# bystrogenomics/bystro-vcf

Hardware: NVIDIA B200
Metric: variants/s (higher is better)
Workload: dtype u8

## Files before the change

### bystro_vcf_b200/csrc/bvcf_api.cu

```cuda
#include "../../include/bvcf.h"

#include <algorithm>
#include <chrono>
#include <cstdio>
#include <cstdlib>
#include <cstring>
#include <string>
#include <vector>

#include "bvcf_common.cuh"
#include "bvcf_prefix.cuh"
#include "bvcf_rows.cuh"
#include "bvcf_tile.cuh"
#include "bvcf_names.cuh"
#include "bvcf_scan.cuh"
#include "bvcf_inflate.cuh"
#include "bvcf_deflate.cuh"

using namespace bvcf;

namespace {

struct DevBuf {
  void *p = nullptr;
// ... 155 lines not shown
  if ((rc = dev_reserve(ctx, sc.tile_base, max_tiles * sizeof(TileBase)))) return rc;
  if ((rc = dev_reserve(ctx, sc.tile_partial, (size_t)TSCAN_BLOCKS * TQ * 8))) return rc;
  sc.scratch_cap = std::max<uint64_t>(sc.scratch_cap, std::min<uint64_t>(total_bytes / 8 + (8ull << 20), sc.max_records * 224ull + (1ull << 20)));
  if ((rc = dev_reserve(ctx, sc.tile_scratch, sc.scratch_cap + 64))) return rc;
  sc.slow_cap = std::max<uint32_t>(sc.slow_cap, 1u << 16);
  if ((rc = dev_reserve(ctx, sc.slow, (size_t)sc.slow_cap * sizeof(SlowRec)))) return rc;
  if (ctx->dcfg.n_samples > 0) {
    sc.row_cap = std::max<uint64_t>(sc.row_cap, sc.max_records / 2 + 1024);
    if ((rc = dev_reserve(ctx, sc.stats1, sc.max_records * sizeof(LineStats)))) return rc;
    if ((rc = dev_reserve(ctx, sc.row_desc, sc.row_cap * sizeof(RowDesc)))) return rc;
    if ((rc = dev_reserve(ctx, sc.big_recs, sc.max_records * 4))) return rc;
  }
  return 0;
}
void scratch_free(Scratch &sc) {
  for (DevBuf *b : {&sc.recs, &sc.range_nrec, &sc.range_nlines, &sc.rec_base, &sc.line_base, &sc.events, &sc.dense,
                    &sc.partial, &sc.stats1, &sc.row_desc, &sc.big_recs, &sc.tile_agg, &sc.tile_base, &sc.tile_partial,
                    &sc.tile_scratch, &sc.slow})
    dev_free(*b);
}

constexpr int N_STAGE_EV = 8;
struct StageEvents {
  cudaEvent_t e[N_STAGE_EV];
};

int enqueue_pipeline(bvcf_ctx *ctx, Scratch &sc, cudaStream_t st, const uint8_t *d_in, uint64_t begin, uint64_t len, uint64_t buf_len,
                     uint8_t *d_out, uint64_t out_cap, RunCounters *d_ctr, int8_t *d_dosage, uint64_t dosage_cap_rows,
                     uint8_t *d_loci, uint64_t loci_cap, unsigned long long *d_loci_off, uint32_t *d_diags,
                     uint32_t diag_cap, std::vector<StageEvents> *timing) {
  const DevCfg &dc = ctx->dcfg;
  const uint64_t a0 = begin & ~511ull;
  const uint64_t total_ranges = (len - a0 + sc.range_bytes - 1) / sc.range_bytes;
  int smem = SCAN_WARPS * RING;
  if (const char *e = getenv("BVCF_SCAN_SMEM_KB")) smem = std::max(smem, atoi(e) * 1024);
  cudaFuncSetAttribute(bvcf_scan_genotype_kernel<true>, cudaFuncAttributeMaxDynamicSharedMemorySize, smem);
  cudaFuncSetAttribute(bvcf_scan_genotype_kernel<false>, cudaFuncAttributeMaxDynamicSharedMemorySize, smem);
  int n_sm = 148;
  cudaDeviceGetAttribute(&n_sm, cudaDevAttrMultiProcessorCount, ctx->device);
  for (uint64_t r0 = 0; r0 < total_ranges; r0 += sc.n_ranges) {
    const uint32_t nr = (uint32_t)std::min<uint64_t>(sc.n_ranges, total_ranges - r0);
    StageEvents *se = nullptr;
    if (timing) {
      timing->emplace_back();
      se = &timing->back();
      for (int i = 0; i < N_STAGE_EV; i++) {
        if (ctx->ev_pool.empty()) {
          cudaEvent_t e;
          CK(cudaEventCreate(&e));
          se->e[i] = e;
        } else {
          se->e[i] = ctx->ev_pool.back();
          ctx->ev_pool.pop_back();
        }
      }
      CK(cudaEventRecord(se->e[0], st));
    }
    ScanParams sp{};
    sp.in = d_in; sp.begin = begin; sp.end = len; sp.buf_len = buf_len; sp.a0 = a0;
    sp.range_bytes = sc.range_bytes; sp.r0 = (uint32_t)r0; sp.n_ranges = nr;
    sp.slots_per_range = sc.slots; sp.evcap_words = sc.evcap_words;
    sp.recs = (LineRec *)sc.recs.p; sp.range_nrec = (uint32_t *)sc.range_nrec.p;
    sp.range_nlines = (uint32_t *)sc.range_nlines.p; sp.events = (uint32_t *)sc.events.p;
    sp.ctr = d_ctr; sp.H = dc.H; sp.eol_width = dc.eol_width;
    const unsigned grid = (nr + SCAN_WARPS - 1) / SCAN_WARPS;
    if (dc.n_samples > 0)
      bvcf_scan_genotype_kernel<true><<<grid, SCAN_WARPS * 32, smem, st>>>(sp);
    else
      bvcf_scan_genotype_kernel<false><<<grid, SCAN_WARPS * 32, smem, st>>>(sp);
    ctx->launches++;
    if (se) CK(cudaEventRecord(se->e[1], st));
    PrefixParams pp{};
    pp.a = sp.range_nrec; pp.b = sp.range_nlines;
    pp.out_a = (uint64_t *)sc.rec_base.p; pp.out_b = (uint64_t *)sc.line_base.p;
    pp.partial = (unsigned long long *)sc.partial.p;
    pp.n_ptr = nullptr; pp.n_imm = nr; pp.ctr = d_ctr;
    bvcf_prefix_reduce_kernel<<<PFX_BLOCKS, PFX_THREADS, 0, st>>>(pp);
    bvcf_prefix_spine_kernel<<<1, 1024, 0, st>>>(pp);
    bvcf_prefix_scan_kernel<<<PFX_BLOCKS, PFX_THREADS, 0, st>>>(pp);
    CompactParams cp{};
    cp.recs = sp.recs; cp.range_nrec = sp.range_nrec; cp.rec_base = pp.out_a; cp.line_base = pp.out_b;
    cp.dense = (LineRec *)sc.dense.p; cp.n_ranges = nr; cp.slots_per_range = sc.slots; cp.evcap_words = sc.evcap_words;
    bvcf_compact_lines_kernel<<<(nr + 7) / 8, 256, 0, st>>>(cp);
    ctx->launches += 4;
    if (se) CK(cudaEventRecord(se->e[2], st));
    const unsigned wgrid = (unsigned)n_sm * 64;
    if (dc.n_samples > 0) {
      StatsParams tp{};
      tp.in = d_in; tp.cfg = dc; tp.lines = cp.dense; tp.events = sp.events; tp.stats = (LineStats *)sc.stats1.p; tp.ctr = d_ctr;
      tp.big_recs = (uint32_t *)sc.big_recs.p;
      bvcf_line_stats_kernel<<<wgrid, 256, 0, st>>>(tp);
      bvcf_line_stats_big_kernel<<<(unsigned)n_sm * 4, 256, 0, st>>>(tp);
      ctx->launches += 2;
    }
    if (se) CK(cudaEventRecord(se->e[3], st));
    static const bool no_vec = getenv("BVCF_NO_NAMES_VEC") != nullptr;
    const bool vec = (dc.name8 || dc.name16) && dc.want_tsv && !no_vec && dc.n_samples > 0;
    TileParams tp{};
    tp.in = d_in; tp.cfg = dc; tp.lines = cp.dense; tp.events = sp.events; tp.stats = (const LineStats *)sc.stats1.p;
    tp.out = d_out; tp.out_cap = out_cap; tp.ctr = d_ctr;
    tp.tile_agg = (TileAgg *)sc.tile_agg.p; tp.tile_base = (TileBase *)sc.tile_base.p;
    tp.tile_partial = (unsigned long long *)sc.tile_partial.p;
    tp.scratch = (uint8_t *)sc.tile_scratch.p; tp.scratch_cap = sc.scratch_cap;
    tp.slow = (SlowRec *)sc.slow.p; tp.slow_cap = sc.slow_cap;
    tp.row_desc = (RowDesc *)sc.row_desc.p; tp.row_desc_cap = dc.n_samples > 0 ? sc.row_cap : 0;
    tp.long_words = vec ? 8192u : 0u;
    {
      static const int mid_q = getenv("BVCF_MID_QUADS") ? atoi(getenv("BVCF_MID_QUADS")) : 16;
      tp.mid_words = (dc.want_tsv && dc.n_samples > 0) ? 2u * (uint32_t)std::max(mid_q, 0) : 0u;
      if (!vec) tp.mid_words = 0;
    }
    tp.dosage = d_dosage; tp.dosage_cap_rows = dosage_cap_rows;
    tp.loci = d_loci; tp.loci_cap = loci_cap; tp.loci_off = d_loci_off;
    tp.diag.diags = d_diags; tp.diag.cap = diag_cap; tp.diag.ctr = d_ctr;
// ... 964 lines not shown
```

### bystro_vcf_b200/csrc/bvcf_common.cuh

```cuda
#pragma once
#include <cstdint>
#include <cuda_runtime.h>

namespace bvcf {

constexpr uint32_t FULL = 0xFFFFFFFFu;

struct __align__(16) LineRec {
  uint64_t start;
  uint32_t len;
  uint32_t an;
  uint32_t ev_start;
  uint32_t ev_count;
  uint32_t ord;
  uint16_t tab[9];
  uint16_t flags;
  uint32_t n_het1, n_hom1, n_miss, ac1;
};
static_assert(sizeof(LineRec) == 64, "LineRec layout");

constexpr uint32_t EV_SAMPLE_MASK = 0xFFFFFu;
constexpr uint32_t EV_COMPLEX = 1u << 30;
constexpr uint32_t EV_OFFSET_TAG = 1u << 31;
constexpr uint32_t EV_CODE_ABSENT = 30, EV_CODE_MISSING = 31;
constexpr uint32_t EV_NIB_MISSING = 0xEu, EV_NIB_ABSENT = 0xFu;
constexpr uint32_t EV_BASE_BIAS = 3;
constexpr uint32_t MAX_SAMPLES = (1u << 20) - 16;

__device__ __forceinline__ uint32_t ev_make(uint32_t sample, uint32_t c1, uint32_t c2) {
  return sample | (c1 << 20) | (c2 << 25);
}
__device__ __forceinline__ uint32_t ev_single_payload(uint32_t c1, uint32_t c2) {
  const uint32_t n1 = c1 == EV_CODE_MISSING ? EV_NIB_MISSING : c1;
  const uint32_t n2 = c2 == EV_CODE_MISSING ? EV_NIB_MISSING : (c2 == EV_CODE_ABSENT ? EV_NIB_ABSENT : c2);
  return n1 | (n2 << 16);
}
__device__ __forceinline__ uint32_t ev_slot_word(uint32_t h, uint32_t pl, int j) {
  const uint32_t samp = (h & EV_SAMPLE_MASK) + (uint32_t)j - EV_BASE_BIAS;
  if (h & EV_COMPLEX) return j == 0 ? (samp | EV_COMPLEX) : EV_OFFSET_TAG;
  const uint32_t n1 = (pl >> (4 * j)) & 0xFu, n2 = (pl >> (16 + 4 * j)) & 0xFu;
  if ((n1 | n2) == 0) return EV_OFFSET_TAG;
  if (n1 == EV_NIB_MISSING || n2 == EV_NIB_MISSING) return ev_make(samp, EV_CODE_MISSING, EV_CODE_MISSING);
  return ev_make(samp, n1, n2 == EV_NIB_ABSENT ? EV_CODE_ABSENT : n2);
}

struct RunCounters {
  unsigned long long out_cursor;
  unsigned long long row_cursor;
  unsigned long long loci_cursor;
  unsigned long long n_lines;
  unsigned long long n_records;
  unsigned long long chunk_out_base;
  unsigned long long chunk_row_base;
  unsigned long long chunk_loci_base;
  unsigned long long chunk_line_base;
  unsigned long long scratch_cursor;
  unsigned int ev_overflow;
  unsigned int slot_overflow;
  unsigned int out_overflow;
  unsigned int row_overflow;
  unsigned int n_diags;
  unsigned int chunk_records;
  unsigned int n_big_recs;
  unsigned int big_rec_cursor;
  unsigned int tile_ticket;
  unsigned int tile_ticket2;
  unsigned int n_slow;
  unsigned int scratch_overflow;
  unsigned int slow_overflow;
  unsigned int n_mid_rows;
  unsigned int n_big_rows;
  unsigned int big_row_cursor;
  unsigned int n_long_rows;
  unsigned int long_row_cursor;
};

struct DevCfg {
  int H;
  int n_samples;
  int eol_width;
  int keep_id, keep_info, keep_pos, want_tsv, want_dosage;
  int allow_all;
  int n_allow, n_excl;
  const uint8_t *filt_blob;
  const uint32_t *filt_off;
  int filt_bytes;
  uint8_t empty[64];
  int empty_len;
  uint8_t delim[64];
  int delim_len;
  uint8_t tail0[208];
  int tail0_len;
  const uint8_t *names;
  const uint32_t *name_off;
  int name_fixed_w;
  const unsigned long long *name8;
  const uint4 *name16;
  int item_bytes;
};

__device__ __forceinline__ uint32_t warp_incl_scan(uint32_t v, int lane) {
#pragma unroll
  for (int d = 1; d < 32; d <<= 1) {
    uint32_t t = __shfl_up_sync(FULL, v, d);
    if (lane >= d) v += t;
  }
  return v;
}
__device__ __forceinline__ uint32_t warp_sum(uint32_t v) {
#pragma unroll
  for (int d = 16; d > 0; d >>= 1) v += __shfl_xor_sync(FULL, v, d);
  return v;
}
__device__ __forceinline__ unsigned long long warp_sum64(unsigned long long v) {
#pragma unroll
  for (int d = 16; d > 0; d >>= 1) v += __shfl_xor_sync(FULL, v, d);
  return v;
}

__device__ __forceinline__ uint32_t eq_mask4(uint32_t w, uint32_t pat) {
  uint32_t t = w ^ pat;
  uint32_t y = (t & 0x7F7F7F7Fu) + 0x7F7F7F7Fu;
  y = ~(y | t | 0x7F7F7F7Fu);
  return ((y >> 7) * 0x00204081u >> 21) & 0xFu;
}
__device__ __forceinline__ uint32_t eq_mask16(const uint4 &v, uint32_t pat) {
  return eq_mask4(v.x, pat) | (eq_mask4(v.y, pat) << 4) | (eq_mask4(v.z, pat) << 8) | (eq_mask4(v.w, pat) << 12);
}

}
```

### bystro_vcf_b200/csrc/bvcf_prefix.cuh

```cuda
#pragma once
#include "bvcf_common.cuh"

namespace bvcf {

constexpr int PFX_BLOCKS = 592;
constexpr int PFX_THREADS = 256;

struct PrefixParams {
  const uint32_t *a, *b;
  uint64_t *out_a, *out_b;
  unsigned long long *partial;
  const unsigned int *n_ptr;
  uint32_t n_imm;
  RunCounters *ctr;
};

__device__ __forceinline__ uint32_t pfx_n(const PrefixParams &p) { return p.n_ptr ? *p.n_ptr : p.n_imm; }

__device__ __forceinline__ void pfx_span(uint32_t n, uint32_t &lo, uint32_t &hi) {
  const uint32_t span = (n + PFX_BLOCKS - 1) / PFX_BLOCKS;
  const unsigned long long l = (unsigned long long)blockIdx.x * span;
  lo = l > n ? n : (uint32_t)l;
  hi = l + span > n ? n : (uint32_t)(l + span);
}
// ... 65 lines not shown
  unsigned long long run_a = p.partial[2 * blockIdx.x], run_b = p.partial[2 * blockIdx.x + 1];
  const int w = threadIdx.x >> 5, l = threadIdx.x & 31;
  for (uint32_t base = lo; base < hi; base += PFX_THREADS) {
    const uint32_t i = base + threadIdx.x;
    const unsigned long long va = i < hi ? p.a[i] : 0, vb = (i < hi && p.b) ? p.b[i] : 0;
    unsigned long long ia = va, ib = vb;
#pragma unroll
    for (int d = 1; d < 32; d <<= 1) {
      const unsigned long long ta = __shfl_up_sync(FULL, ia, d), tb = __shfl_up_sync(FULL, ib, d);
      if (l >= d) { ia += ta; ib += tb; }
    }
    __syncthreads();
    if (l == 31) { wa[w] = ia; wb[w] = ib; }
    __syncthreads();
    unsigned long long oa = 0, ob = 0, ta = 0, tb = 0;
#pragma unroll
    for (int k = 0; k < PFX_THREADS / 32; k++) {
      if (k < w) { oa += wa[k]; ob += wb[k]; }
      ta += wa[k]; tb += wb[k];
    }
    if (i < hi) {
      p.out_a[i] = run_a + oa + ia - va;
      if (p.out_b) p.out_b[i] = run_b + ob + ib - vb;
    }
    run_a += ta; run_b += tb;
  }
}

struct CompactParams {
  const LineRec *recs;
  const uint32_t *range_nrec;
  const uint64_t *rec_base;
  const uint64_t *line_base;
  LineRec *dense;
  uint32_t n_ranges, slots_per_range, evcap_words;
};

__global__ void __launch_bounds__(256) bvcf_compact_lines_kernel(const CompactParams p) {
  const uint32_t r = blockIdx.x * 8 + (threadIdx.x >> 5);
  const int lane = threadIdx.x & 31;
  if (r >= p.n_ranges) return;
  uint32_t n = p.range_nrec[r];
  if (n > p.slots_per_range) n = p.slots_per_range;
  const LineRec *src = p.recs + (size_t)r * p.slots_per_range;
  LineRec *dst = p.dense + p.rec_base[r];
  const uint32_t lb = (uint32_t)p.line_base[r];
  for (uint32_t j = lane; j < n; j += 32) {
    LineRec x = src[j];
    x.ev_start += r * p.evcap_words;
    x.ord += lb;
    dst[j] = x;
  }
}

}
```

### bystro_vcf_b200/csrc/bvcf_rows.cuh

```cuda
#pragma once
#include "bvcf_common.cuh"
#include "bvcf_text.cuh"

namespace bvcf {

constexpr int NAMES_WARPS = 2;
constexpr int FILT_SMEM = 1024;

struct GtStats {
  uint32_t n_het, n_hom, n_miss, ac, an;
  uint32_t het_bytes, hom_bytes, miss_bytes;
};

constexpr int STAT_ALLELES = 3;
struct __align__(16) LineStats {
  uint32_t n_miss, an, miss_bytes, pad;
  uint32_t n_het[STAT_ALLELES], n_hom[STAT_ALLELES], ac[STAT_ALLELES], het_bytes[STAT_ALLELES], hom_bytes[STAT_ALLELES];
  uint32_t pad2;
};

struct __align__(16) RowDesc {
  uint32_t line;
  uint32_t allele;
  unsigned long long het_dst, hom_dst, miss_dst;
// ... 87 lines not shown
  const uint32_t q = v >> 2;
  off = 0;
  if (2 * q + 1 >= n_words) return EV_OFFSET_TAG;
  const uint2 e = *reinterpret_cast<const uint2 *>(ev + 2 * q);
  off = e.y;
  return ev_slot_word(e.x, e.y, (int)(v & 3u));
}

__device__ __forceinline__ int classify_word(uint32_t w, uint32_t off, const uint8_t *L,
                                             uint32_t content_len, uint32_t a, uint32_t &samp, uint32_t &gt_extra,
                                             uint32_t &alt) {
  gt_extra = 0; alt = 0; samp = 0;
  if (w & EV_OFFSET_TAG) return 0;
  samp = w & EV_SAMPLE_MASK;
  if (w & EV_COMPLEX) {
    uint32_t gt;
    const int cls = classify_gt_general(L + off, content_len > off ? content_len - off : 0, a, gt, alt);
    gt_extra = gt;
    return cls;
  }
  const uint32_t c1 = (w >> 20) & 31, c2 = (w >> 25) & 31;
  if (c1 == EV_CODE_MISSING) return 3;
  alt = (c1 == a) + (c2 == a);
  const uint32_t gt = c2 == EV_CODE_ABSENT ? 1 : 2;
  return alt == 0 ? 0 : (alt == gt ? 2 : 1);
}
__device__ __forceinline__ int classify_event(const uint32_t *ev, uint32_t v, uint32_t n_words, const uint8_t *L,
                                              uint32_t content_len, uint32_t a, uint32_t &samp, uint32_t &gt_extra,
                                              uint32_t &alt, bool &is_ev) {
  uint32_t off;
  const uint32_t w = slot_load(ev, v, n_words, off);
  is_ev = !(w & EV_OFFSET_TAG);
  return classify_word(w, off, L, content_len, a, samp, gt_extra, alt);
}

__device__ __forceinline__ uint32_t nib_eq(uint32_t x, uint32_t pat) {
  const uint32_t y = x ^ pat;
  return ~(((y & 0x77777777u) + 0x77777777u) | y) & 0x88888888u;
}

__device__ __forceinline__ void quad_masks(uint32_t h, uint32_t pl, uint32_t a, bool simple, const uint8_t *L,
                                           uint32_t content_len, bool valid, uint32_t &mh, uint32_t &mo, uint32_t &mm) {
  mh = mo = mm = 0;
  if (!valid) return;
  uint32_t one1, one2, dot, hap;
  if (simple) {
    const uint32_t b0 = pl << 3, b3 = pl;
    const uint32_t one = b0 & ~b3 & 0x88888888u, dt = b3 & ~b0 & 0x88888888u;
    one1 = one & 0x8888u; one2 = one >> 16;
    dot = dt | (dt >> 16);
    hap = (b3 & b0 & 0x88888888u) >> 16;
  } else {
    if (h & EV_COMPLEX) {
      uint32_t gt, alt;
      const int cls = classify_gt_general(L + pl, content_len > pl ? content_len - pl : 0, a, gt, alt);
      if (cls == 1) mh = 8u; else if (cls == 2) mo = 8u; else if (cls == 3) mm = 8u;
      return;
    }
    const uint32_t eq = a <= 9 ? nib_eq(pl, a * 0x11111111u) : 0u;
    const uint32_t dt = nib_eq(pl, 0xEEEEEEEEu);
    one1 = eq & 0x8888u; one2 = eq >> 16;
    dot = dt | (dt >> 16);
    hap = nib_eq(pl, 0xFFFFFFFFu) >> 16;
  }
  mm = dot & 0x8888u;
  mo = one1 & (one2 | hap) & ~mm;
  mh = (one1 ^ one2) & ~hap & ~mm & 0x8888u;
}

struct StatsParams {
  const uint8_t *in;
// ... 567 lines not shown
```

### bystro_vcf_b200/csrc/bvcf_scan.cuh

```cuda
#pragma once
#include "bvcf_common.cuh"

namespace bvcf {

constexpr int WIN = 512;
constexpr int STAGES = 8;
constexpr int RING = WIN * STAGES;
constexpr int PF_PAIRS = 3;
constexpr int SCAN_WARPS = 8;
constexpr int FS_NONE = 0x7FFFFFFF;

struct ScanParams {
  const uint8_t *in;
  uint64_t begin, end;
  uint64_t buf_len;
  uint64_t a0;
  uint32_t range_bytes;
  uint32_t r0, n_ranges;
  uint32_t slots_per_range, evcap_words;
  LineRec *recs;
  uint32_t *range_nrec;
  uint32_t *range_nlines;
  uint32_t *events;
  RunCounters *ctr;
  int H, eol_width;
};

struct LineAcc {
  uint32_t an_l, an_uni;
  uint32_t het_l, hom_l;
  uint32_t ac_l;
  uint32_t miss_l;
  uint32_t flag_l;
};

struct WarpState {
  uint64_t line_start;
  int fsr;
  uint32_t col;
  uint32_t ev_w, line_ev_start;
  uint32_t nrec, nlines;
  uint32_t refpat;
  int mode;
  LineAcc a;
};

__device__ __forceinline__ uint4 lds128(uint32_t a) {
  uint4 v;
  asm volatile("ld.shared.v4.u32 {%0,%1,%2,%3}, [%4];\n" : "=r"(v.x), "=r"(v.y), "=r"(v.z), "=r"(v.w) : "r"(a));
  return v;
}
__device__ __forceinline__ uint32_t lds32(uint32_t a) {
  uint32_t v;
  asm volatile("ld.shared.u32 %0, [%1];\n" : "=r"(v) : "r"(a));
  return v;
}

__device__ __forceinline__ uint32_t bits_range16(int lo, int hi) {
  lo = lo < 0 ? 0 : lo;
  hi = hi > 16 ? 16 : hi;
  return hi <= lo ? 0u : (((1u << hi) - 1u) & ~((1u << lo) - 1u));
}

__device__ __forceinline__ uint32_t tok_code(uint32_t c) {
  uint32_t d = c - '0';
  return c == '.' ? EV_CODE_MISSING : (d <= 9 ? d : 0u);
}

__device__ __forceinline__ void start_line(WarpState &st, uint64_t start, int rel) {
  st.line_start = start; st.fsr = rel; st.col = 0;
  st.a.an_l = st.a.an_uni = st.a.het_l = st.a.hom_l = st.a.ac_l = st.a.miss_l = st.a.flag_l = 0;
  st.line_ev_start = st.ev_w;
}

__device__ __forceinline__ void acc_sample(LineAcc &a, uint32_t c1, uint32_t c2) {
  const uint32_t hap = c2 == EV_CODE_ABSENT;
  const uint32_t alt = (c1 == 1) + (c2 == 1);
  a.ac_l += alt;
  a.hom_l += hap ? alt : (alt >> 1);
  a.het_l += hap ? 0u : (alt & 1u);
  a.flag_l |= (c1 > 1) | (!hap && c2 > 1);
}

__device__ __forceinline__ uint32_t pack_quad(const uint32_t t[4], bool dots) {
  if (dots) {
    const uint32_t K = 0x000F000Fu;
    return (t[0] & K) | ((t[1] & K) << 4) | ((t[2] & K) << 8) | ((t[3] & K) << 12);
  }
  return t[0] | (t[1] << 4) | (t[2] << 8) | (t[3] << 12);
}
__device__ __forceinline__ void acc_quad(LineAcc &a, uint32_t pl, bool dots) {
  const uint32_t y = pl ^ 0x11111111u;
  uint32_t one = ~(((y & 0x77777777u) + 0x77777777u) | y) & 0x88888888u;
  uint32_t big = pl & 0xEEEEEEEEu;
  if (dots) {
    const uint32_t d = pl ^ 0xEEEEEEEEu;
    const uint32_t dot = ~(((d & 0x77777777u) + 0x77777777u) | d) & 0x88888888u;
    const uint32_t mf = (dot | (dot >> 16)) & 0x8888u;
    const uint32_t nm = __popc(mf);
    a.miss_l += nm;
    a.an_l -= 2 * nm;
    const uint32_t gone = ((mf | (mf << 16)) >> 3) * 15u;
    one &= ~gone;
    big &= ~gone;
  }
  const uint32_t both = one & (one >> 16);
  const uint32_t n1 = __popc(one), n2 = __popc(both);
  a.ac_l += n1;
  a.hom_l += n2;
  a.het_l += n1 - 2 * n2;
  a.flag_l |= big;
}
__device__ __forceinline__ void classify_push_words4(const ScanParams &p, WarpState &st, uint32_t *my_events,
                                                     const uint32_t t[4], int samp0, bool dots, int lane) {
  const uint32_t pl = pack_quad(t, dots);
  const uint32_t bal = __ballot_sync(FULL, pl != 0);
  if (bal == 0) return;
  const uint32_t n = 2 * __popc(bal);
  if (st.ev_w + n <= p.evcap_words) {
    if (pl)
      *reinterpret_cast<uint2 *>(my_events + st.ev_w + 2 * __popc(bal & ((1u << lane) - 1u))) =
          make_uint2((uint32_t)(samp0 + (int)EV_BASE_BIAS), pl);
  } else if (lane == 0) {
    p.ctr->ev_overflow = 1;
  }
  if (pl) acc_quad(st.a, pl, dots);
  st.ev_w += n;
}

__device__ __forceinline__ void classify_push_pair(const ScanParams &p, WarpState &st, uint32_t *my_events,
                                                   const uint32_t ta[4], const uint32_t tb[4], int samp0, bool dots,
                                                   int lane) {
  const uint32_t pa = pack_quad(ta, dots), pb = pack_quad(tb, dots);
  const uint32_t ba = __ballot_sync(FULL, pa != 0), bb = __ballot_sync(FULL, pb != 0);
  if ((ba | bb) == 0) return;
  const uint32_t na = 2 * __popc(ba), n = na + 2 * __popc(bb);
  const uint32_t lt = (1u << lane) - 1u;
  if (st.ev_w + n <= p.evcap_words) {
    uint32_t *dst = my_events + st.ev_w;
    if (pa) *reinterpret_cast<uint2 *>(dst + 2 * __popc(ba & lt)) = make_uint2((uint32_t)(samp0 + (int)EV_BASE_BIAS), pa);
    if (pb)
      *reinterpret_cast<uint2 *>(dst + na + 2 * __popc(bb & lt)) = make_uint2((uint32_t)(samp0 + 128 + (int)EV_BASE_BIAS), pb);
  } else if (lane == 0) {
    p.ctr->ev_overflow = 1;
  }
  if (pa) acc_quad(st.a, pa, dots);
  if (pb) acc_quad(st.a, pb, dots);
  st.ev_w += n;
}

__device__ __forceinline__ uint32_t bad_digits4(const uint32_t t[4], uint32_t keep_mask3) {
  const uint32_t o = t[0] | t[1] | t[2] | (t[3] & keep_mask3);
  return (o & 0xFFF0FFF0u) | (((o & 0x000F000Fu) + 0x00060006u) & 0x00100010u);
}
__device__ __forceinline__ uint32_t bad_digits8(const uint32_t ta[4], const uint32_t tb[4]) {
  const uint32_t o = ta[0] | ta[1] | ta[2] | ta[3] | tb[0] | tb[1] | tb[2] | tb[3];
  return (o & 0xFFF0FFF0u) | (((o & 0x000F000Fu) + 0x00060006u) & 0x00100010u);
}
__device__ __forceinline__ uint32_t bad_digits_or_dots4(const uint32_t t[4], uint32_t keep_mask3) {
  const uint32_t o = t[0] | t[1] | t[2] | (t[3] & keep_mask3);
  uint32_t acc = 0;
#pragma unroll
  for (int j = 0; j < 4; j++) {
    const uint32_t x = t[j] + 0x00160016u, y = t[j] + 0x00020002u, z = t[j] + 0x00010001u;
    acc |= (x & ~y) | z;
  }
  return (o & 0xFFE0FFE0u) | (acc & 0x00200020u);
}

template <bool HAS_SAMPLES>
__device__ __forceinline__ void scan_window_general(const ScanParams &p, WarpState &st, uint32_t ring_base_s,
                                                    uint32_t stage_off, const uint4 &v, uint64_t pos, uint64_t rend,
                                                    int lane, LineRec *my_recs, uint32_t *my_events) {
  const bool eol2 = p.eol_width == 2;
  const uint32_t tm = eq_mask16(v, 0x09090909u);
  uint32_t nm = eq_mask16(v, 0x0A0A0A0Au);

  int seg_lo = 0;
  if (st.mode == 1 && st.fsr != FS_NONE && st.fsr > 0) {
    seg_lo = st.fsr;
    nm &= bits_range16(seg_lo - lane * 16, 16);
  }

  while (seg_lo < WIN) {
    const int lo_l = seg_lo - lane * 16;
    const uint32_t ball = __ballot_sync(FULL, nm != 0);
    int nl = WIN;
    if (ball) {
      const int l = __ffs(ball) - 1;
      const uint32_t m = __shfl_sync(FULL, nm, l);
      nl = l * 16 + __ffs(m) - 1;
      if (lane == l) nm &= nm - 1;
    }
    if (st.mode == 0) {
      if (nl == WIN) return;
      const uint64_t start = pos + nl + 1;
      if (start >= rend) { st.mode = 2; return; }
      st.mode = 1;
      start_line(st, start, nl + 1);
      seg_lo = nl + 1;
      continue;
    }
    int tab_hi = nl;
    if (eol2 && nl < WIN && nl > 0) tab_hi = nl - 1;
    const uint32_t tm_l = tm & bits_range16(lo_l, tab_hi - lane * 16);
    const uint32_t cnt = __popc(tm_l);
// ... 66 lines not shown
            bad_shape = true;
          }
        }
        uint32_t bad = bad_digits4(t, 0xFFFFFFFFu) | (bad_shape ? 1u : 0u);
        bool dots = false;
        if (!__all_sync(FULL, bad == 0)) {
          bad = bad_digits_or_dots4(t, 0xFFFFFFFFu) | (bad_shape ? 1u : 0u);
          dots = true;
        }
        if (__all_sync(FULL, bad == 0)) {
          vector_ok = true;
          const int samp0 = (int)samp_base + ((ws0 - s9) >> 2);
          st.a.an_l += 2 * __popc(zone);
          classify_push_words4(p, st, my_events, t, samp0, dots, lane);
          if (nl == WIN) {
            const int n_words = (WIN - s9 + 3) >> 2;
            const int ws_last = s9 + 4 * (n_words - 1);
            nfs = ws_last + 4 - WIN;
            col_extra = ws_last + 3 >= WIN ? 1u : 0u;
          }
        }
      }
      if (!vector_ok) {
        if (!have_excl) excl = warp_incl_scan(cnt, lane) - cnt;
        int last_end = -1;
        uint32_t last_sep = 0;
        const uint32_t prev_hi = __shfl_up_sync(FULL, tm_l >> 15, 1);
        uint32_t fm = ((tm_l << 1) | (lane > 0 ? (prev_hi & 1u) : 0u)) & 0xFFFFu;
        if (st.fsr == seg_lo) {
          const int sl = seg_lo - lane * 16;
          if (sl >= 0 && sl < 16) fm |= 1u << sl;
        }
        const uint32_t fm_all = fm;
        uint32_t evbuf[16];
        int nev = 0;
        while (fm) {
          const int sl = __ffs(fm) - 1;
          fm &= fm - 1;
          const uint32_t fidx = st.col + excl + __popc(tm_l & ((1u << sl) - 1u));
          last_end = -1;
          if (fidx < 9) continue;
          const uint32_t samp = fidx - 9;
          const int s = lane * 16 + sl;
          const uint32_t a = stage_off + (uint32_t)s;
          const uint32_t w0 = lds32(ring_base_s + ((a & ~3u) & (RING - 1)));
          const uint32_t w1 = lds32(ring_base_s + (((a & ~3u) + 4u) & (RING - 1)));
          const uint32_t sh = (a & 3u) * 8u;
          const uint32_t lo = __funnelshift_r(w0, w1, sh);
          const uint32_t b0 = lo & 0xFF, b1 = (lo >> 8) & 0xFF, b2 = (lo >> 16) & 0xFF, b3 = lo >> 24;
          const uint32_t b4 = (w1 >> sh) & 0xFF;
          auto is_end = [&](uint32_t c, uint32_t nx) { return c == '\t' || c == '\n' || c == ':' || (eol2 && nx == '\n'); };
          auto is_sep = [](uint32_t c) { return c == '|' || c == '/'; };
          const bool e0 = is_end(b0, b1), e1 = is_end(b1, b2), e2 = is_end(b2, b3), e3 = is_end(b3, b4);
          if (e0) {
            st.a.an_l += 1;
            if (b0 == '\t') last_end = s;
          } else if (!is_sep(b0) && e1) {
            const uint32_t c = tok_code(b0);
            if (c == EV_CODE_MISSING) {
              evbuf[nev++] = samp + EV_BASE_BIAS; evbuf[nev++] = ev_single_payload(EV_CODE_MISSING, EV_CODE_MISSING);
              st.a.miss_l++;
            } else {
              st.a.an_l += 1;
              if (c) {
                evbuf[nev++] = samp + EV_BASE_BIAS; evbuf[nev++] = ev_single_payload(c, EV_CODE_ABSENT);
                acc_sample(st.a, c, EV_CODE_ABSENT);
              }
            }
            if (b1 == '\t') last_end = s + 1;
          } else if (!is_sep(b0) && is_sep(b1) && !e2 && !is_sep(b2) && e3) {
            const uint32_t c1 = tok_code(b0), c2 = tok_code(b2);
            if (c1 == EV_CODE_MISSING || c2 == EV_CODE_MISSING) {
              evbuf[nev++] = samp + EV_BASE_BIAS; evbuf[nev++] = ev_single_payload(EV_CODE_MISSING, EV_CODE_MISSING);
              st.a.miss_l++;
            } else {
              st.a.an_l += 2;
              if (c1 | c2) {
                evbuf[nev++] = samp + EV_BASE_BIAS; evbuf[nev++] = ev_single_payload(c1, c2);
                acc_sample(st.a, c1, c2);
              }
            }
            if (b3 == '\t') { last_end = s + 3; last_sep = b1; }
          } else {
            evbuf[nev++] = (samp + EV_BASE_BIAS) | EV_COMPLEX;
            evbuf[nev++] = (uint32_t)(pos + (uint64_t)s - st.line_start);
            st.a.flag_l |= 1;
          }
        }
        const uint32_t eincl = warp_incl_scan((uint32_t)nev, lane);
        const uint32_t etot = __shfl_sync(FULL, eincl, 31);
        if (etot) {
          if (st.ev_w + etot <= p.evcap_words) {
            uint32_t *dst = my_events + st.ev_w + (eincl - nev);
            for (int k = 0; k < nev; k++) dst[k] = evbuf[k];
          } else if (lane == 0) {
            p.ctr->ev_overflow = 1;
          }
          st.ev_w += etot;
        }
        if (nl == WIN) {
          const uint32_t last_tab = __shfl_sync(FULL, tm_l >> 15, 31) & 1u;
          if (last_tab) {
            nfs = 0;
          } else {
            const uint32_t have = __ballot_sync(FULL, fm_all != 0);
            if (have) {
              const int l = 31 - __clz(have);
              const int le = __shfl_sync(FULL, last_end, l);
              const uint32_t sp = __shfl_sync(FULL, last_sep, l);
              if (le >= WIN) {
                nfs = le + 1 - WIN; col_extra = 1;
                if (sp) st.refpat = 0x09300030u | (sp << 8);
              }
            }
          }
        }
      }
    }
    st.col += total;

    if (nl < WIN) {
      st.nlines++;
      const LineAcc &a = st.a;
      const uint32_t an = __reduce_add_sync(FULL, a.an_l) + a.an_uni;
      uint32_t n_het = 0, n_hom = 0, n_miss = 0, ac = 0, flag = 0;
      if (HAS_SAMPLES) {
        flag = __any_sync(FULL, a.flag_l != 0);
        if (__any_sync(FULL, (a.het_l | a.hom_l | a.miss_l) != 0)) {
          n_het = __reduce_add_sync(FULL, a.het_l); n_hom = __reduce_add_sync(FULL, a.hom_l);
          ac = __reduce_add_sync(FULL, a.ac_l); n_miss = __reduce_add_sync(FULL, a.miss_l);
        }
      }
      if (st.col == (uint32_t)(p.H - 1)) {
        if (st.nrec < p.slots_per_range) {
          if (lane == 0) {
            LineRec *r = &my_recs[st.nrec];
            r->start = st.line_start;
            r->len = (uint32_t)(pos + nl + 1 - st.line_start);
            r->an = an;
            r->ev_start = st.line_ev_start;
            r->ev_count = st.ev_w - st.line_ev_start;
            r->ord = st.nlines - 1;
            r->flags = (uint16_t)flag;
            r->n_het1 = n_het; r->n_hom1 = n_hom; r->n_miss = n_miss; r->ac1 = ac;
          }
        } else if (lane == 0) {
          p.ctr->slot_overflow = 1;
        }
        st.nrec++;
      } else {
        st.ev_w = st.line_ev_start;
      }
      const uint64_t start = pos + nl + 1;
      if (start >= rend) { st.mode = 2; return; }
      start_line(st, start, nl + 1);
      seg_lo = nl + 1;
      continue;
    }
    st.col += col_extra;
    st.fsr = nfs;
    return;
  }
  if (st.mode == 1) st.fsr = seg_lo - WIN;
}

template <bool HAS_SAMPLES>
__global__ void __launch_bounds__(SCAN_WARPS * 32) bvcf_scan_genotype_kernel(const ScanParams p) {
  extern __shared__ __align__(16) uint8_t smem[];
  const int warp = threadIdx.x >> 5, lane = threadIdx.x & 31;
  const uint32_t rl = blockIdx.x * SCAN_WARPS + warp;
  if (rl >= p.n_ranges) return;
  const uint64_t rstart = p.a0 + (uint64_t)(p.r0 + rl) * p.range_bytes;
  uint64_t rend = rstart + p.range_bytes;
  if (rend > p.end) rend = p.end;
  LineRec *my_recs = p.recs + (size_t)rl * p.slots_per_range;
  uint32_t *my_events = p.events + (size_t)rl * p.evcap_words;

  WarpState st;
  st.nrec = 0; st.nlines = 0; st.ev_w = 0;
  st.refpat = 0x09307C30u;
  st.mode = 0;
  start_line(st, 0, FS_NONE);
  if (rstart >= p.end) {
    st.mode = 2;
  } else if (rstart <= p.begin) {
    st.mode = 1; st.line_start = p.begin; st.fsr = (int)(p.begin - rstart);
  } else if (p.in[rstart - 1] == '\n') {
    st.mode = 1; st.line_start = rstart; st.fsr = 0;
  }

  if (st.mode != 2) {
    const uint32_t ring_base_s = (uint32_t)__cvta_generic_to_shared(smem + warp * RING);
    const uint32_t ring_lane_s = ring_base_s + lane * 16;
    const uint64_t avail64 = (p.buf_len - rstart) / WIN;
    const uint32_t n_avail = avail64 > 0xFFFFFFF0ull ? 0xFFFFFFF0u : (uint32_t)avail64;
    const uint32_t seek_limit = (uint32_t)((rend - rstart + WIN - 1) / WIN);
    const uint8_t *gsrc = p.in + rstart + lane * 16;
    uint32_t issue_off = 0;
    auto issue_pair = [&]() {
      const uint32_t d = ring_lane_s + issue_off;
      asm volatile("cp.async.cg.shared.global [%0], [%1], 16;\n" ::"r"(d), "l"(gsrc));
      asm volatile("cp.async.cg.shared.global [%0], [%1], 16;\n" ::"r"(d + WIN), "l"(gsrc + WIN));
      asm volatile("cp.async.commit_group;\n" ::);
      gsrc += 2 * WIN;
      issue_off = (issue_off + 2 * WIN) & (RING - 1);
    };
#pragma unroll
    for (int k = 0; k < PF_PAIRS; k++) issue_pair();
    uint32_t stage_off = 0;
    bool done = false;
    bool fast = HAS_SAMPLES && st.mode == 1 && st.col >= 9 && (uint32_t)st.fsr < 4u;
    for (uint32_t it = 0; it + 2 < n_avail && !done; it += 2, stage_off = (stage_off + 2 * WIN) & (RING - 1)) {
      issue_pair();
      asm volatile("cp.async.wait_group %0;\n" ::"n"(PF_PAIRS - 1));
      __syncwarp();
      int hint = 0;
      if (fast) {
        const uint32_t rp = st.refpat;
        const uint32_t sh = (uint32_t)st.fsr * 8u;
        const uint32_t rot = __funnelshift_l(rp, rp, sh);
        uint4 va, vb;
        uint32_t w4b;
        bool allref;
        for (;;) {
          const uint32_t so_b = (stage_off + WIN) & (RING - 1);
          va = lds128(ring_lane_s + stage_off);
// ... 46 lines not shown
        const uint32_t so = (stage_off + h * WIN) & (RING - 1);
        if (st.mode == 0 && wi >= seek_limit) { done = true; break; }
        const uint4 v = lds128(ring_lane_s + so);
        if (st.mode == 0) {
          const uint32_t K = 0x7F7F7F7Fu;
          const uint32_t a = v.x ^ 0x0A0A0A0Au, b = v.y ^ 0x0A0A0A0Au, c = v.z ^ 0x0A0A0A0Au, d = v.w ^ 0x0A0A0A0Au;
          const uint32_t z = ~((((a & K) + K) | a) & (((b & K) + K) | b) & (((c & K) + K) | c) & (((d & K) + K) | d)) & ~K;
          if (!__any_sync(FULL, z != 0)) continue;
        }
        if (fast && hint != 2 - h) {
          const uint32_t w4 = lds32(ring_base_s + ((so + lane * 16 + 16) & (RING - 1)));
          const uint32_t sh = (uint32_t)st.fsr * 8u;
          const uint32_t rp = st.refpat;
          const uint32_t t[4] = {__funnelshift_r(v.x, v.y, sh) ^ rp, __funnelshift_r(v.y, v.z, sh) ^ rp,
                                 __funnelshift_r(v.z, v.w, sh) ^ rp, __funnelshift_r(v.w, w4, sh) ^ rp};
          if (__all_sync(FULL, (t[0] | t[1] | t[2] | t[3]) == 0)) {
            st.a.an_uni += 256; st.col += 128;
            continue;
          }
          uint32_t bad = bad_digits4(t, 0xFFFFFFFFu);
          bool dots = false;
          if (!__all_sync(FULL, bad == 0)) {
            bad = bad_digits_or_dots4(t, 0xFFFFFFFFu);
            dots = true;
          }
          if (__all_sync(FULL, bad == 0)) {
            st.a.an_uni += 256;
            classify_push_words4(p, st, my_events, t, (int)(st.col - 9) + lane * 4, dots, lane);
            st.col += 128;
            continue;
          }
        }
        const uint64_t pos = rstart + (uint64_t)wi * WIN;
        scan_window_general<HAS_SAMPLES>(p, st, ring_base_s, so, v, pos, rend, lane, my_recs, my_events);
        if (st.mode == 2) { done = true; break; }
        fast = HAS_SAMPLES && st.mode == 1 && st.col >= 9 && (uint32_t)st.fsr < 4u;
      }
      __syncwarp();
    }
  }
  asm volatile("cp.async.wait_group 0;\n" ::);
  if (lane == 0) {
    p.range_nrec[rl] = st.nrec < p.slots_per_range ? st.nrec : p.slots_per_range;
    p.range_nlines[rl] = st.nlines;
  }
}

}
```

### bystro_vcf_b200/csrc/bvcf_tile.cuh

```cuda
#pragma once
#include "bvcf_rows.cuh"

namespace bvcf {

constexpr int TILE_THREADS = 32;
constexpr int TILE_WARPS = 4;
constexpr uint32_t TILE_ROWS_MAX = 160;
constexpr uint32_t ROW_NONE = 0xFFFFu;

struct __align__(16) TRow {
  uint32_t hole_len[3];
  uint16_t hole_pos[3];
  uint16_t soff;
  uint16_t slen;
  uint16_t loc_len;
  uint16_t next;
  uint16_t allele;
  uint16_t flags;
  uint16_t pad;
};
static_assert(sizeof(TRow) == 32, "TRow layout");

struct __align__(16) LaneRec {
  unsigned long long bytes;
// ... 22 lines not shown
struct __align__(16) SlowRec {
  unsigned long long out_off, loci_off;
  uint32_t li, row, desc, flags;
};

struct TileParams {
  const uint8_t *in;
  DevCfg cfg;
  const LineRec *lines;
  const uint32_t *events;
  const LineStats *stats;
  uint8_t *out;
  unsigned long long out_cap;
  RunCounters *ctr;
  TileAgg *tile_agg;
  TileBase *tile_base;
  unsigned long long *tile_partial;
  uint8_t *scratch;
  unsigned long long scratch_cap;
  SlowRec *slow;
  uint32_t slow_cap;
  RowDesc *row_desc;
  unsigned long long row_desc_cap;
  uint32_t mid_words, long_words;
  int8_t *dosage;
  unsigned long long dosage_cap_rows;
  uint8_t *loci;
  unsigned long long loci_cap;
  unsigned long long *loci_off;
  DiagSink diag;
};

__device__ __forceinline__ void sts8(uint32_t a, uint32_t v) { asm volatile("st.shared.u8 [%0], %1;\n" ::"r"(a), "r"(v)); }
__device__ __forceinline__ void sts32(uint32_t a, uint32_t v) { asm volatile("st.shared.u32 [%0], %1;\n" ::"r"(a), "r"(v)); }
__device__ __forceinline__ void store_head(uint8_t *&g, unsigned long long &v, uint32_t &n, uint32_t &moved) {
  moved = 0;
  if (((uintptr_t)g & 1u) && n >= 1) { *g = (uint8_t)v; v >>= 8; g += 1; n -= 1; moved += 1; }
  if (((uintptr_t)g & 2u) && n >= 2) { *reinterpret_cast<uint16_t *>(g) = (uint16_t)v; v >>= 16; g += 2; n -= 2; moved += 2; }
  if (((uintptr_t)g & 4u) && n >= 4) { *reinterpret_cast<uint32_t *>(g) = (uint32_t)v; v >>= 32; g += 4; n -= 4; moved += 4; }
}
__device__ __forceinline__ void store_tail(uint8_t *g, unsigned long long v, uint32_t n) {
  if (n & 4u) { *reinterpret_cast<uint32_t *>(g) = (uint32_t)v; v >>= 32; g += 4; }
  if (n & 2u) { *reinterpret_cast<uint16_t *>(g) = (uint16_t)v; v >>= 16; g += 2; }
  if (n & 1u) *g = (uint8_t)v;
}
__device__ __forceinline__ unsigned long long ldg64_unaligned(const uint8_t *s) { return ld64_any(s); }

__device__ __forceinline__ void copy_g2g(uint8_t *__restrict__ g_, const uint8_t *__restrict__ s_, uint32_t n) {
  if (n == 0) return;
  uint8_t *g = g_;
  const uint8_t *s = s_;
  if ((uintptr_t)g & 7u) {
    unsigned long long v = ldg64_unaligned(s);
    if (n < 8 && (((uintptr_t)g & 7u) + n) <= 8u) {
      for (uint32_t i = 0; i < n; i++) g[i] = (uint8_t)(v >> (8 * i));
      return;
    }
    uint32_t moved;
    store_head(g, v, n, moved);
    s += moved;
  }
  if (n >= 8) {
    const uint32_t sh = (uint32_t)((uintptr_t)s & 3u) * 8u;
    const uint32_t *__restrict__ wp = reinterpret_cast<const uint32_t *>((uintptr_t)s & ~(uintptr_t)3);
    uint32_t w0 = wp[0];
    while (n >= 32) {
      const uint32_t w1 = wp[1], w2 = wp[2], w3 = wp[3], w4 = wp[4], w5 = wp[5], w6 = wp[6], w7 = wp[7], w8 = wp[8];
// ... 1169 lines not shown
```

Measured before the change: 282.7 million.

## Move per-line genotype stats from scan kernel into compact kernel

The scan kernel no longer accumulates het/hom/missing/AC/flag counts per line. The compaction kernel now recomputes them from the stored event words using nibble-parallel bit tricks, with a warp-cooperative path for lines that have many events. The per-lane local evbuf array is moved into dynamic shared memory, and launch bounds add a minimum-blocks hint, both aimed at cutting register pressure and raising occupancy of the hot scan kernel. The cost is that the compact kernel must re-read the event data, and the larger shared-memory footprint may limit resident blocks.

```diff
diff --git a/bystro_vcf_b200/csrc/bvcf_api.cu b/bystro_vcf_b200/csrc/bvcf_api.cu
--- a/bystro_vcf_b200/csrc/bvcf_api.cu
+++ b/bystro_vcf_b200/csrc/bvcf_api.cu
@@ -211,10 +211,10 @@
   const DevCfg &dc = ctx->dcfg;
   const uint64_t a0 = begin & ~511ull;
   const uint64_t total_ranges = (len - a0 + sc.range_bytes - 1) / sc.range_bytes;
-  int smem = SCAN_WARPS * RING;
+  int smem = scan_smem(dc.n_samples > 0);
   if (const char *e = getenv("BVCF_SCAN_SMEM_KB")) smem = std::max(smem, atoi(e) * 1024);
-  cudaFuncSetAttribute(bvcf_scan_genotype_kernel<true>, cudaFuncAttributeMaxDynamicSharedMemorySize, smem);
-  cudaFuncSetAttribute(bvcf_scan_genotype_kernel<false>, cudaFuncAttributeMaxDynamicSharedMemorySize, smem);
+  cudaFuncSetAttribute(dc.n_samples > 0 ? bvcf_scan_genotype_kernel<true> : bvcf_scan_genotype_kernel<false>,
+                       cudaFuncAttributeMaxDynamicSharedMemorySize, smem);
   int n_sm = 148;
   cudaDeviceGetAttribute(&n_sm, cudaDevAttrMultiProcessorCount, ctx->device);
   for (uint64_t r0 = 0; r0 < total_ranges; r0 += sc.n_ranges) {
@@ -259,6 +259,7 @@
     bvcf_prefix_scan_kernel<<<PFX_BLOCKS, PFX_THREADS, 0, st>>>(pp);
     CompactParams cp{};
     cp.recs = sp.recs; cp.range_nrec = sp.range_nrec; cp.rec_base = pp.out_a; cp.line_base = pp.out_b;
+    cp.events = sp.events; cp.ctr = d_ctr;
     cp.dense = (LineRec *)sc.dense.p; cp.n_ranges = nr; cp.slots_per_range = sc.slots; cp.evcap_words = sc.evcap_words;
     bvcf_compact_lines_kernel<<<(nr + 7) / 8, 256, 0, st>>>(cp);
     ctx->launches += 4;
diff --git a/bystro_vcf_b200/csrc/bvcf_common.cuh b/bystro_vcf_b200/csrc/bvcf_common.cuh
--- a/bystro_vcf_b200/csrc/bvcf_common.cuh
+++ b/bystro_vcf_b200/csrc/bvcf_common.cuh
@@ -42,6 +42,11 @@
   if ((n1 | n2) == 0) return EV_OFFSET_TAG;
   if (n1 == EV_NIB_MISSING || n2 == EV_NIB_MISSING) return ev_make(samp, EV_CODE_MISSING, EV_CODE_MISSING);
   return ev_make(samp, n1, n2 == EV_NIB_ABSENT ? EV_CODE_ABSENT : n2);
+}
+
+__device__ __forceinline__ uint32_t nib_eq(uint32_t x, uint32_t pat) {
+  const uint32_t y = x ^ pat;
+  return ~(((y & 0x77777777u) + 0x77777777u) | y) & 0x88888888u;
 }
 
 struct RunCounters {
@@ -99,6 +104,8 @@
   int item_bytes;
 };
 
+__device__ __forceinline__ void sts32(uint32_t a, uint32_t v) { asm volatile("st.shared.u32 [%0], %1;\n" ::"r"(a), "r"(v)); }
+
 __device__ __forceinline__ uint32_t warp_incl_scan(uint32_t v, int lane) {
 #pragma unroll
   for (int d = 1; d < 32; d <<= 1) {
diff --git a/bystro_vcf_b200/csrc/bvcf_prefix.cuh b/bystro_vcf_b200/csrc/bvcf_prefix.cuh
--- a/bystro_vcf_b200/csrc/bvcf_prefix.cuh
+++ b/bystro_vcf_b200/csrc/bvcf_prefix.cuh
@@ -121,9 +121,31 @@
   const uint32_t *range_nrec;
   const uint64_t *rec_base;
   const uint64_t *line_base;
+  const uint32_t *events;
+  const RunCounters *ctr;
   LineRec *dense;
   uint32_t n_ranges, slots_per_range, evcap_words;
 };
+
+struct Alt1Sum {
+  uint32_t het, hom, miss, ac, flag;
+};
+__device__ __forceinline__ void alt1_quad(Alt1Sum &s, uint2 e) {
+  if (e.x & EV_COMPLEX) { s.flag = 1; return; }
+  const uint32_t pl = e.y;
+  const uint32_t dot = nib_eq(pl, 0xEEEEEEEEu), absent = nib_eq(pl, 0xFFFFFFFFu), one = nib_eq(pl, 0x11111111u);
+  const uint32_t ms = (dot | (dot >> 16)) & 0x8888u;
+  const uint32_t gone = ((ms | (ms << 16)) >> 3) * 15u;
+  const uint32_t hap = (absent >> 16) & ~ms;
+  const uint32_t one1 = one & ~gone & 0x8888u, one2 = (one & ~gone) >> 16;
+  s.miss += __popc(ms);
+  s.ac += __popc(one1) + __popc(one2);
+  s.hom += __popc(one1 & (one2 | hap));
+  s.het += __popc((one1 ^ one2) & ~hap);
+  s.flag |= pl & ~gone & ~((absent >> 3) * 15u) & 0xEEEEEEEEu;
+}
+
+constexpr uint32_t ALT1_LANE_WORDS = 32;
 
 __global__ void __launch_bounds__(256) bvcf_compact_lines_kernel(const CompactParams p) {
   const uint32_t r = blockIdx.x * 8 + (threadIdx.x >> 5);
@@ -133,12 +155,38 @@
   if (n > p.slots_per_range) n = p.slots_per_range;
   const LineRec *src = p.recs + (size_t)r * p.slots_per_range;
   LineRec *dst = p.dense + p.rec_base[r];
+  const uint32_t *ev = p.events + (size_t)r * p.evcap_words;
   const uint32_t lb = (uint32_t)p.line_base[r];
-  for (uint32_t j = lane; j < n; j += 32) {
-    LineRec x = src[j];
-    x.ev_start += r * p.evcap_words;
-    x.ord += lb;
-    dst[j] = x;
+  const bool ev_ok = !p.ctr->ev_overflow;
+  for (uint32_t j0 = 0; j0 < n; j0 += 32) {
+    const uint32_t j = j0 + lane;
+    const bool valid = j < n;
+    LineRec x;
+    x.ev_start = 0; x.ev_count = 0;
+    if (valid) x = src[j];
+    Alt1Sum s{0, 0, 0, 0, 0};
+    const bool lane_sum = valid && ev_ok && x.ev_count <= ALT1_LANE_WORDS;
+    if (lane_sum)
+      for (uint32_t q = 0; 2 * q + 1 < x.ev_count; q++) alt1_quad(s, *reinterpret_cast<const uint2 *>(ev + x.ev_start + 2 * q));
+    uint32_t big = __ballot_sync(FULL, valid && ev_ok && !lane_sum);
+    while (big) {
+      const int l = __ffs(big) - 1;
+      big &= big - 1;
+      const uint32_t es = __shfl_sync(FULL, x.ev_start, l), nq = __shfl_sync(FULL, x.ev_count, l) >> 1;
+      Alt1Sum w{0, 0, 0, 0, 0};
+      for (uint32_t q = lane; q < nq; q += 32) alt1_quad(w, *reinterpret_cast<const uint2 *>(ev + es + 2 * q));
+      const uint32_t het = __reduce_add_sync(FULL, w.het), hom = __reduce_add_sync(FULL, w.hom);
+      const uint32_t miss = __reduce_add_sync(FULL, w.miss), ac = __reduce_add_sync(FULL, w.ac);
+      const uint32_t flag = __any_sync(FULL, w.flag != 0);
+      if (lane == l) { s.het = het; s.hom = hom; s.miss = miss; s.ac = ac; s.flag = flag; }
+    }
+    if (valid) {
+      x.ev_start += r * p.evcap_words;
+      x.ord += lb;
+      x.flags = s.flag ? 1 : 0;
+      x.n_het1 = s.het; x.n_hom1 = s.hom; x.n_miss = s.miss; x.ac1 = s.ac;
+      dst[j] = x;
+    }
   }
 }
 
diff --git a/bystro_vcf_b200/csrc/bvcf_rows.cuh b/bystro_vcf_b200/csrc/bvcf_rows.cuh
--- a/bystro_vcf_b200/csrc/bvcf_rows.cuh
+++ b/bystro_vcf_b200/csrc/bvcf_rows.cuh
@@ -143,11 +143,6 @@
   const uint32_t w = slot_load(ev, v, n_words, off);
   is_ev = !(w & EV_OFFSET_TAG);
   return classify_word(w, off, L, content_len, a, samp, gt_extra, alt);
-}
-
-__device__ __forceinline__ uint32_t nib_eq(uint32_t x, uint32_t pat) {
-  const uint32_t y = x ^ pat;
-  return ~(((y & 0x77777777u) + 0x77777777u) | y) & 0x88888888u;
 }
 
 __device__ __forceinline__ void quad_masks(uint32_t h, uint32_t pl, uint32_t a, bool simple, const uint8_t *L,
diff --git a/bystro_vcf_b200/csrc/bvcf_scan.cuh b/bystro_vcf_b200/csrc/bvcf_scan.cuh
--- a/bystro_vcf_b200/csrc/bvcf_scan.cuh
+++ b/bystro_vcf_b200/csrc/bvcf_scan.cuh
@@ -8,6 +8,8 @@
 constexpr int RING = WIN * STAGES;
 constexpr int PF_PAIRS = 3;
 constexpr int SCAN_WARPS = 8;
+constexpr int EVBUF = 16 * 32 * 4;
+constexpr int scan_smem(bool has_samples) { return SCAN_WARPS * (RING + (has_samples ? EVBUF : 0)); }
 constexpr int FS_NONE = 0x7FFFFFFF;
 
 struct ScanParams {
@@ -28,10 +30,6 @@
 
 struct LineAcc {
   uint32_t an_l, an_uni;
-  uint32_t het_l, hom_l;
-  uint32_t ac_l;
-  uint32_t miss_l;
-  uint32_t flag_l;
 };
 
 struct WarpState {
@@ -69,17 +67,8 @@
 
 __device__ __forceinline__ void start_line(WarpState &st, uint64_t start, int rel) {
   st.line_start = start; st.fsr = rel; st.col = 0;
-  st.a.an_l = st.a.an_uni = st.a.het_l = st.a.hom_l = st.a.ac_l = st.a.miss_l = st.a.flag_l = 0;
+  st.a.an_l = st.a.an_uni = 0;
   st.line_ev_start = st.ev_w;
-}
-
-__device__ __forceinline__ void acc_sample(LineAcc &a, uint32_t c1, uint32_t c2) {
-  const uint32_t hap = c2 == EV_CODE_ABSENT;
-  const uint32_t alt = (c1 == 1) + (c2 == 1);
-  a.ac_l += alt;
-  a.hom_l += hap ? alt : (alt >> 1);
-  a.het_l += hap ? 0u : (alt & 1u);
-  a.flag_l |= (c1 > 1) | (!hap && c2 > 1);
 }
 
 __device__ __forceinline__ uint32_t pack_quad(const uint32_t t[4], bool dots) {
@@ -89,27 +78,10 @@
   }
   return t[0] | (t[1] << 4) | (t[2] << 8) | (t[3] << 12);
 }
-__device__ __forceinline__ void acc_quad(LineAcc &a, uint32_t pl, bool dots) {
-  const uint32_t y = pl ^ 0x11111111u;
-  uint32_t one = ~(((y & 0x77777777u) + 0x77777777u) | y) & 0x88888888u;
-  uint32_t big = pl & 0xEEEEEEEEu;
-  if (dots) {
-    const uint32_t d = pl ^ 0xEEEEEEEEu;
-    const uint32_t dot = ~(((d & 0x77777777u) + 0x77777777u) | d) & 0x88888888u;
-    const uint32_t mf = (dot | (dot >> 16)) & 0x8888u;
-    const uint32_t nm = __popc(mf);
-    a.miss_l += nm;
-    a.an_l -= 2 * nm;
-    const uint32_t gone = ((mf | (mf << 16)) >> 3) * 15u;
-    one &= ~gone;
-    big &= ~gone;
-  }
-  const uint32_t both = one & (one >> 16);
-  const uint32_t n1 = __popc(one), n2 = __popc(both);
-  a.ac_l += n1;
-  a.hom_l += n2;
-  a.het_l += n1 - 2 * n2;
-  a.flag_l |= big;
+__device__ __forceinline__ void an_drop_missing(LineAcc &a, uint32_t pl) {
+  const uint32_t d = pl ^ 0xEEEEEEEEu;
+  const uint32_t dot = ~(((d & 0x77777777u) + 0x77777777u) | d) & 0x88888888u;
+  a.an_l -= 2 * __popc((dot | (dot >> 16)) & 0x8888u);
 }
 __device__ __forceinline__ void classify_push_words4(const ScanParams &p, WarpState &st, uint32_t *my_events,
                                                      const uint32_t t[4], int samp0, bool dots, int lane) {
@@ -124,7 +96,7 @@
   } else if (lane == 0) {
     p.ctr->ev_overflow = 1;
   }
-  if (pl) acc_quad(st.a, pl, dots);
+  if (dots && pl) an_drop_missing(st.a, pl);
   st.ev_w += n;
 }
 
@@ -144,8 +116,10 @@
   } else if (lane == 0) {
     p.ctr->ev_overflow = 1;
   }
-  if (pa) acc_quad(st.a, pa, dots);
-  if (pb) acc_quad(st.a, pb, dots);
+  if (dots) {
+    if (pa) an_drop_missing(st.a, pa);
+    if (pb) an_drop_missing(st.a, pb);
+  }
   st.ev_w += n;
 }
 
@@ -170,8 +144,8 @@
 
 template <bool HAS_SAMPLES>
 __device__ __forceinline__ void scan_window_general(const ScanParams &p, WarpState &st, uint32_t ring_base_s,
-                                                    uint32_t stage_off, const uint4 &v, uint64_t pos, uint64_t rend,
-                                                    int lane, LineRec *my_recs, uint32_t *my_events) {
+                                                    uint32_t stage_off, uint32_t evbuf_s, const uint4 &v, uint64_t pos,
+                                                    uint64_t rend, int lane, LineRec *my_recs, uint32_t *my_events) {
   const bool eol2 = p.eol_width == 2;
   const uint32_t tm = eq_mask16(v, 0x09090909u);
   uint32_t nm = eq_mask16(v, 0x0A0A0A0Au);
@@ -304,8 +278,12 @@
           if (sl >= 0 && sl < 16) fm |= 1u << sl;
         }
         const uint32_t fm_all = fm;
-        uint32_t evbuf[16];
         int nev = 0;
+        auto push_ev = [&](uint32_t w0, uint32_t w1) {
+          sts32(evbuf_s + (uint32_t)(nev * 32 + lane) * 4u, w0);
+          sts32(evbuf_s + (uint32_t)(nev * 32 + 32 + lane) * 4u, w1);
+          nev += 2;
+        };
         while (fm) {
           const int sl = __ffs(fm) - 1;
           fm &= fm - 1;
@@ -330,33 +308,23 @@
           } else if (!is_sep(b0) && e1) {
             const uint32_t c = tok_code(b0);
             if (c == EV_CODE_MISSING) {
-              evbuf[nev++] = samp + EV_BASE_BIAS; evbuf[nev++] = ev_single_payload(EV_CODE_MISSING, EV_CODE_MISSING);
-              st.a.miss_l++;
+              push_ev(samp + EV_BASE_BIAS, ev_single_payload(EV_CODE_MISSING, EV_CODE_MISSING));
             } else {
               st.a.an_l += 1;
-              if (c) {
-                evbuf[nev++] = samp + EV_BASE_BIAS; evbuf[nev++] = ev_single_payload(c, EV_CODE_ABSENT);
-                acc_sample(st.a, c, EV_CODE_ABSENT);
-              }
+              if (c) push_ev(samp + EV_BASE_BIAS, ev_single_payload(c, EV_CODE_ABSENT));
             }
             if (b1 == '\t') last_end = s + 1;
           } else if (!is_sep(b0) && is_sep(b1) && !e2 && !is_sep(b2) && e3) {
             const uint32_t c1 = tok_code(b0), c2 = tok_code(b2);
             if (c1 == EV_CODE_MISSING || c2 == EV_CODE_MISSING) {
-              evbuf[nev++] = samp + EV_BASE_BIAS; evbuf[nev++] = ev_single_payload(EV_CODE_MISSING, EV_CODE_MISSING);
-              st.a.miss_l++;
+              push_ev(samp + EV_BASE_BIAS, ev_single_payload(EV_CODE_MISSING, EV_CODE_MISSING));
             } else {
               st.a.an_l += 2;
-              if (c1 | c2) {
-                evbuf[nev++] = samp + EV_BASE_BIAS; evbuf[nev++] = ev_single_payload(c1, c2);
-                acc_sample(st.a, c1, c2);
-              }
+              if (c1 | c2) push_ev(samp + EV_BASE_BIAS, ev_single_payload(c1, c2));
             }
             if (b3 == '\t') { last_end = s + 3; last_sep = b1; }
           } else {
-            evbuf[nev++] = (samp + EV_BASE_BIAS) | EV_COMPLEX;
-            evbuf[nev++] = (uint32_t)(pos + (uint64_t)s - st.line_start);
-            st.a.flag_l |= 1;
+            push_ev((samp + EV_BASE_BIAS) | EV_COMPLEX, (uint32_t)(pos + (uint64_t)s - st.line_start));
           }
         }
         const uint32_t eincl = warp_incl_scan((uint32_t)nev, lane);
@@ -364,7 +332,7 @@
         if (etot) {
           if (st.ev_w + etot <= p.evcap_words) {
             uint32_t *dst = my_events + st.ev_w + (eincl - nev);
-            for (int k = 0; k < nev; k++) dst[k] = evbuf[k];
+            for (int k = 0; k < nev; k++) dst[k] = lds32(evbuf_s + (uint32_t)(k * 32 + lane) * 4u);
           } else if (lane == 0) {
             p.ctr->ev_overflow = 1;
           }
@@ -393,16 +361,7 @@
 
     if (nl < WIN) {
       st.nlines++;
-      const LineAcc &a = st.a;
-      const uint32_t an = __reduce_add_sync(FULL, a.an_l) + a.an_uni;
-      uint32_t n_het = 0, n_hom = 0, n_miss = 0, ac = 0, flag = 0;
-      if (HAS_SAMPLES) {
-        flag = __any_sync(FULL, a.flag_l != 0);
-        if (__any_sync(FULL, (a.het_l | a.hom_l | a.miss_l) != 0)) {
-          n_het = __reduce_add_sync(FULL, a.het_l); n_hom = __reduce_add_sync(FULL, a.hom_l);
-          ac = __reduce_add_sync(FULL, a.ac_l); n_miss = __reduce_add_sync(FULL, a.miss_l);
-        }
-      }
+      const uint32_t an = __reduce_add_sync(FULL, st.a.an_l) + st.a.an_uni;
       if (st.col == (uint32_t)(p.H - 1)) {
         if (st.nrec < p.slots_per_range) {
           if (lane == 0) {
@@ -413,8 +372,6 @@
             r->ev_start = st.line_ev_start;
             r->ev_count = st.ev_w - st.line_ev_start;
             r->ord = st.nlines - 1;
-            r->flags = (uint16_t)flag;
-            r->n_het1 = n_het; r->n_hom1 = n_hom; r->n_miss = n_miss; r->ac1 = ac;
           }
         } else if (lane == 0) {
           p.ctr->slot_overflow = 1;
@@ -437,7 +394,7 @@
 }
 
 template <bool HAS_SAMPLES>
-__global__ void __launch_bounds__(SCAN_WARPS * 32) bvcf_scan_genotype_kernel(const ScanParams p) {
+__global__ void __launch_bounds__(SCAN_WARPS * 32, HAS_SAMPLES ? 4 : 5) bvcf_scan_genotype_kernel(const ScanParams p) {
   extern __shared__ __align__(16) uint8_t smem[];
   const int warp = threadIdx.x >> 5, lane = threadIdx.x & 31;
   const uint32_t rl = blockIdx.x * SCAN_WARPS + warp;
@@ -464,6 +421,7 @@
   if (st.mode != 2) {
     const uint32_t ring_base_s = (uint32_t)__cvta_generic_to_shared(smem + warp * RING);
     const uint32_t ring_lane_s = ring_base_s + lane * 16;
+    const uint32_t evbuf_s = (uint32_t)__cvta_generic_to_shared(smem + SCAN_WARPS * RING + warp * EVBUF);
     const uint64_t avail64 = (p.buf_len - rstart) / WIN;
     const uint32_t n_avail = avail64 > 0xFFFFFFF0ull ? 0xFFFFFFF0u : (uint32_t)avail64;
     const uint32_t seek_limit = (uint32_t)((rend - rstart + WIN - 1) / WIN);
@@ -576,7 +534,7 @@
           }
         }
         const uint64_t pos = rstart + (uint64_t)wi * WIN;
-        scan_window_general<HAS_SAMPLES>(p, st, ring_base_s, so, v, pos, rend, lane, my_recs, my_events);
+        scan_window_general<HAS_SAMPLES>(p, st, ring_base_s, so, evbuf_s, v, pos, rend, lane, my_recs, my_events);
         if (st.mode == 2) { done = true; break; }
         fast = HAS_SAMPLES && st.mode == 1 && st.col >= 9 && (uint32_t)st.fsr < 4u;
       }
diff --git a/bystro_vcf_b200/csrc/bvcf_tile.cuh b/bystro_vcf_b200/csrc/bvcf_tile.cuh
--- a/bystro_vcf_b200/csrc/bvcf_tile.cuh
+++ b/bystro_vcf_b200/csrc/bvcf_tile.cuh
@@ -78,7 +78,6 @@
 };
 
 __device__ __forceinline__ void sts8(uint32_t a, uint32_t v) { asm volatile("st.shared.u8 [%0], %1;\n" ::"r"(a), "r"(v)); }
-__device__ __forceinline__ void sts32(uint32_t a, uint32_t v) { asm volatile("st.shared.u32 [%0], %1;\n" ::"r"(a), "r"(v)); }
 __device__ __forceinline__ void store_head(uint8_t *&g, unsigned long long &v, uint32_t &n, uint32_t &moved) {
   moved = 0;
   if (((uintptr_t)g & 1u) && n >= 1) { *g = (uint8_t)v; v >>= 8; g += 1; n -= 1; moved += 1; }
```

Result: no change. 282.4 million, median of 6 (-0.1%).
